# mrvollger/rustybam

Hardware: AMD Instinct MI355X
Metric: CIGAR-ops/s, liftover over 100 kb sliding windows (whole pass, inputs resident in HBM) (higher is better)
Workload: dtype u32

## Files before the change

### rustybam_amd/csrc/capi.hip

```cpp
#include <hip/hip_runtime.h>
#include <sys/mman.h>

#include <algorithm>
#include <cstdarg>
#include <cstdio>
#include <cstdlib>
#include <cstring>
#include <ctime>
#include <numeric>
#include <string>
#include <thread>
#include <vector>
#include <chrono>
#include <map>
#include <mutex>

#include "../../include/rustybam_amd.h"
#include "rb_lift.h"
#include "rb_trim.h"
#include "rb_launch.h"

#ifndef RB_SCAN_ROWS_MEAN_MAX
#define RB_SCAN_ROWS_MEAN_MAX 1536
#endif
#ifndef RB_SHORT_MAX_DEFAULT
#define RB_SHORT_MAX_DEFAULT 2048
#endif

#define RB_MAX_ARENA 256

#define RB_TIMING_RING 256
__global__ __launch_bounds__(256) void rb_k_fill_bytes(uint8_t *dst, uint32_t v4, size_t n) {
    const uintptr_t a = (uintptr_t)dst;
    const size_t head = n < 16 ? n : (size_t)((16 - (a & 15)) & 15);
    const size_t body = (n - head) / 16;
    const size_t tail0 = head + body * 16;
    const size_t i = (size_t)blockIdx.x * blockDim.x + threadIdx.x, stride = (size_t)gridDim.x * blockDim.x;
    for (size_t k = i; k < body; k += stride) *reinterpret_cast<uint4 *>(dst + head + k * 16) = make_uint4(v4, v4, v4, v4);
    if (i < head) dst[i] = (uint8_t)v4;
    if (i < n - tail0) dst[tail0 + i] = (uint8_t)v4;
}
extern "C" hipError_t rb_fill_async(void *dst, int value, size_t bytes, hipStream_t stream) {
    if (!bytes) return hipSuccess;
    const uint32_t b = (uint32_t)value & 255u, v4 = b | (b << 8) | (b << 16) | (b << 24);
// ... 22 lines not shown
    bool pin_busy[2] = {false, false};
    unsigned pin_next = 0;
    uint64_t alloc_fallbacks = 0;
    struct cached_buf { void *p; size_t bytes; bool placed; };
    std::vector<cached_buf> cache;
    size_t cache_bytes = 0;
};
#define RB_PIN_CHUNK ((size_t)32 << 20)
#define RB_PIN_MIN ((size_t)8 << 20)

struct rb_plan {
    rb_ctx *ctx = nullptr;
    uint64_t n_rec = 0, n_win = 0, n_ops = 0;
    uint32_t n_contig = 0;
    uint32_t depth = 0;
    uint32_t *sched = nullptr, *slot_of = nullptr, *canon_pos = nullptr, *w_orig = nullptr, *ident = nullptr;
    uint64_t *w_st = nullptr, *w_en = nullptr, *wo_st = nullptr, *wo_en = nullptr, *cw_off = nullptr;
    uint8_t *cw_mono = nullptr;
    uint32_t *tiles = nullptr;
    uint32_t n_tiles = 0, stream_end = 0;
};

static int fail(rb_ctx *ctx, int code, const char *fmt, ...) {
    if (ctx) {
        char buf[512];
        va_list ap;
        va_start(ap, fmt);
        vsnprintf(buf, sizeof buf, fmt, ap);
        va_end(ap);
        ctx->err = buf;
    }
// ... 496 lines not shown

extern "C" int rb_plan_create(rb_ctx *ctx, uint64_t n_rec, const uint64_t *op_off, const uint32_t *contig, uint64_t n_win,
                              const uint32_t *w_contig, const uint64_t *w_st, const uint64_t *w_en, rb_plan **out) {
    if (!ctx || !out || (n_rec && (!op_off || !contig))) return RB_E_INVALID;
    if (n_rec >= 0xFFFFFFFFull || n_win >= 0xFFFFFFFFull) return fail(ctx, RB_E_INVALID, "too many records/windows for one batch");
    HIPCHK(ctx, hipSetDevice(ctx->device));
    rb_plan *pl = new rb_plan();
    pl->ctx = ctx;
    pl->n_rec = n_rec;
    pl->n_win = n_win;
    uint32_t maxc = 0;
    for (uint64_t i = 0; i < n_rec; i++) maxc = std::max(maxc, contig[i]);
    for (uint64_t i = 0; i < n_win; i++) maxc = std::max(maxc, w_contig[i]);
    const uint32_t n_contig = (n_rec || n_win) ? maxc + 1 : 0;
    pl->n_contig = n_contig;
    std::vector<uint32_t> canon_pos(n_rec);
    {
        std::vector<uint64_t> rank(n_contig, UINT64_MAX);
        uint64_t nr = 0;
        for (uint64_t i = 0; i < n_rec; i++)
            if (rank[contig[i]] == UINT64_MAX) rank[contig[i]] = nr++;
        std::vector<uint64_t> start(nr + 1, 0);
        for (uint64_t i = 0; i < n_rec; i++) start[rank[contig[i]] + 1]++;
        for (uint64_t k = 0; k < nr; k++) start[k + 1] += start[k];
        for (uint64_t i = 0; i < n_rec; i++) canon_pos[i] = (uint32_t)start[rank[contig[i]]]++;
    }
    std::vector<uint32_t> sched(n_rec), ident(n_rec);
    std::iota(ident.begin(), ident.end(), 0u);
    {
        uint64_t max_len = 0;
        std::vector<uint64_t> key(n_rec);
        for (uint64_t i = 0; i < n_rec; i++) key[i] = op_off[i + 1] - op_off[i], max_len = std::max(max_len, key[i]);
        int passes = 0;
        while (passes < 4 && (max_len >> (16 * passes)) != 0) passes++;
        std::vector<uint32_t> a(ident), b(n_rec);
        std::vector<uint64_t> cnt(65537);
        for (int ps = 0; ps < passes; ps++) {
            std::fill(cnt.begin(), cnt.end(), 0);
            const int sh = 16 * ps;
            for (uint64_t i = 0; i < n_rec; i++) cnt[(0xFFFFu - (uint32_t)((key[i] >> sh) & 0xFFFFu)) + 1]++;
// ... 43 lines not shown
        if (const char *m = getenv("RB_SHORT_MAX")) short_max = strtoull(m, nullptr, 10);
        if (on && n_rec) {
            uint64_t n_long = 0;
            rb_cut_tiles(n_rec, op_off, short_max, sched, tiles, &n_long);
            if (!tiles.empty()) pl->stream_end = (uint32_t)n_long;
        }
        pl->n_tiles = (uint32_t)(tiles.size() / 3);
    }
    int rc = RB_OK;
    std::vector<uint32_t> slot_of(n_rec);
    for (uint64_t w = 0; w < n_rec; w++) slot_of[sched[w]] = (uint32_t)w;
    if (!rc) rc = upload_vec(ctx, sched, &pl->sched);
    if (!rc) rc = upload_vec(ctx, slot_of, &pl->slot_of);
    if (!rc) rc = upload_vec(ctx, ident, &pl->ident);
    if (!rc) rc = upload_vec(ctx, canon_pos, &pl->canon_pos);
    if (!rc) rc = upload_vec(ctx, g_st, &pl->w_st);
    if (!rc) rc = upload_vec(ctx, g_en, &pl->w_en);
    if (!rc) rc = upload_vec(ctx, g_orig, &pl->w_orig);
    if (!rc) rc = upload_vec(ctx, o_st, &pl->wo_st);
    if (!rc) rc = upload_vec(ctx, o_en, &pl->wo_en);
    if (!rc) rc = upload_vec(ctx, cw_off, &pl->cw_off);
    if (!rc) rc = upload_vec(ctx, mono, &pl->cw_mono);
    if (!rc && pl->n_tiles) rc = upload_vec(ctx, tiles, &pl->tiles);
    if (!rc && hipStreamSynchronize(ctx->stream) != hipSuccess) rc = fail(ctx, RB_E_HIP, "plan upload: %s", hipGetErrorString(hipGetLastError()));
    if (rc) {
        rb_plan_destroy(pl);
        return rc;
    }
    *out = pl;
    return RB_OK;
}
extern "C" void rb_plan_destroy(rb_plan *pl) {
    if (!pl) return;
    void *ptrs[] = {pl->sched, pl->slot_of, pl->ident, pl->canon_pos, pl->w_st, pl->w_en, pl->w_orig, pl->wo_st, pl->wo_en, pl->cw_off, pl->cw_mono, pl->tiles};
    for (void *q : ptrs)
        if (q) (void)rb_dev_free(pl->ctx, q);
    delete pl;
}

struct ws_layout {
    size_t hit_off, win_lo, block_sums, arena, pend_count, pend_list, jobs, gen_list, x_st, x_en, bp_tmp, bp_off, bp_cur, brk_rows, copy_count, copy_list, decl_count, decl_list, gen_cp, diag_stamps, fb_count, fb_list, starts_bad, total;
};
static bool rb_no_gen_cp() {
    static const bool v = getenv("RB_DEBUG_NO_GEN_CP") != nullptr;
    return v;
}
static ws_layout ws_of(uint64_t n_rec, uint64_t rows_cap, uint64_t n_ops) {
    ws_layout w;
    size_t o = 0;
    auto take = [&](size_t bytes) {
        size_t at = o;
        o += (bytes + 255) & ~(size_t)255;
        return at;
    };
    w.hit_off = take((n_rec + 2) * 8);
    w.win_lo = take((n_rec + 2) * 4);
// ... 6 lines not shown
    w.x_st = take((rows_cap + 1) * 8);
    w.x_en = take((rows_cap + 1) * 8);
    w.bp_tmp = take((rows_cap + 1) * 8);
    w.bp_off = take((n_rec + 1) * 8);
    w.bp_cur = take((size_t)RB_MAX_ARENA * 128);
    w.brk_rows = take((rows_cap + 1) * sizeof(rb_hit_row));
    w.copy_count = take(256);
    w.copy_list = take((rows_cap + 1) * 16);
    w.decl_count = take(256);
    w.decl_list = take((n_rec + 1) * 4);
    w.gen_cp = take(rb_no_gen_cp() ? 256 : (size_t)(n_ops / RB_GCP + n_rec + 2) * sizeof(uint4));
    w.diag_stamps = take((n_rec + 1) * 4);
    w.fb_count = take(256);
    w.fb_list = take((n_rec + 1) * 4);
    w.starts_bad = take(256);
    w.total = o;
    return w;
}
extern "C" size_t rb_plan_workspace_bytes(const rb_plan *plan, uint64_t rows_cap) {
    if (!plan) return 0;
    return ws_of(plan->n_rec, rows_cap, plan->n_ops).total;
}
extern "C" size_t rb_plan_diag_stamps_offset(const rb_plan *plan, uint64_t rows_cap) {
    if (!plan) return 0;
    return ws_of(plan->n_rec, rows_cap, plan->n_ops).diag_stamps;
}

static uint64_t slot_stride_of(uint64_t n_ops, uint64_t n_rec) { return ((n_ops + 31) & ~(uint64_t)31) + 32 * n_rec + 64; }
extern "C" uint64_t rb_plan_out_capacity(const rb_plan *plan, int for_break) {
    if (!plan) return 0;
// ... 76 lines not shown
        HIPCHK(ctx, hipMemcpyAsync(&first_bad, bad, 8, hipMemcpyDeviceToHost, ctx->stream));
        HIPCHK(ctx, hipStreamSynchronize(ctx->stream));
        if (first_bad != ~0ull)
            return fail(ctx, RB_E_INVALID, "RB_LIFT_OP_STARTS: record %llu lies outside the batch's %llu ops (a pass moved it: gather the batch first)",
                        first_bad, (unsigned long long)b->n_ops);
    }
    p.norm_w = const_cast<rb_norm_row *>(norm);
    p.pend_list = (uint32_t *)(ws + w.pend_list);
    p.pend_count = (unsigned long long *)(ws + w.pend_count);
    const bool use_tiles = plan->n_tiles != 0 && ((policy >> 8) & 0xFFF) == 0;
    p.tile_first = use_tiles ? plan->tiles : nullptr;
    p.n_tiles = use_tiles ? plan->n_tiles : 0;
    p.fb_list = (uint32_t *)(ws + w.fb_list);
    p.fb_count = (unsigned long long *)(ws + w.fb_count);
    const uint32_t stream_end = use_tiles ? plan->stream_end : (uint32_t)b->n_rec;
    rb_scan_params sp;
    memset(&sp, 0, sizeof sp);
    if (p.fused) {
        sp.n_rec = b->n_rec;
        sp.ops = b->ops;
        sp.op_off = b->op_off;
        sp.t_st = b->t_st, sp.t_en = b->t_en, sp.q_st = b->q_st, sp.q_en = b->q_en;
        sp.strand = b->strand;
        sp.norm_rows = p.norm_w;
        HIPCHK(ctx, rb_fill_async(p.pend_count, 0, 8, ctx->stream));
        HIPCHK(ctx, rb_launch_peek_norm(&sp, ctx->stream));
    }
    p.counters = counters;
    p.policy = policy & 1;
    p.early_exit = (policy & RB_LIFT_EARLY_EXIT) ? 1 : 0;
    p.debug_skip = (policy >> 8) & 0xFFF;
    uint64_t *block_sums = (uint64_t *)(ws + w.block_sums);
    HIPCHK(ctx, rb_fill_async(counters, 0, sizeof(rb_counters), ctx->stream));
    HIPCHK(ctx, rb_fill_async(p.copy_count, 0, 8, ctx->stream));
    HIPCHK(ctx, rb_fill_async(p.arena_cur, 0, (size_t)RB_MAX_ARENA * RB_ARENA_STRIDE * 8, ctx->stream));
    if (b->n_rec == 0) return RB_OK;
    const bool one_walk = is_break && (policy & RB_BREAK_ONE_WALK) && !p.desc_mode;
    if (one_walk) {
        p.brk_mode = 1, p.brk_max = max_size;
        p.rows_final = rows;
        p.rows = (rb_hit_row *)(ws + w.brk_rows);
        p.brk_off = (uint64_t *)(ws + w.bp_off);
        p.brk_cursor = (unsigned long long *)(ws + w.bp_cur);
        p.brk_n_arena = pick_arenas(b->n_rec);
        p.brk_arena_cap = rows_cap / p.brk_n_arena;
        p.brk_decl_list = (uint32_t *)(ws + w.decl_list);
        p.brk_decl_count = (unsigned long long *)(ws + w.decl_count);
        HIPCHK(ctx, rb_fill_async(p.brk_decl_count, 0, 8, ctx->stream));
        HIPCHK(ctx, rb_fill_async(p.brk_cursor, 0, (size_t)RB_MAX_ARENA * 128, ctx->stream));
        HIPCHK(ctx, rb_fill_async(p.hit_off, 0, (size_t)(b->n_rec + 2) * 8, ctx->stream));
        HIPCHK(ctx, rb_fill_async(p.brk_off, 0xFF, (size_t)(b->n_rec + 1) * 8, ctx->stream));
        HIPCHK(ctx, rb_launch_make_jobs(&p, ctx->stream));
        const size_t slot1 = (size_t)(ctx->timed_calls % RB_TIMING_RING);
        if (ctx->timing) HIPCHK(ctx, hipEventRecord(ctx->ev_a[slot1], ctx->stream));
        p.wave0 = 0;
        p.wave_end = stream_end;
        HIPCHK(ctx, rb_launch_liftover_stream(&p, ctx->stream));
        if (use_tiles) {
            HIPCHK(ctx, rb_fill_async(p.fb_count, 0, 8, ctx->stream));
            HIPCHK(ctx, rb_launch_liftover_tiles(&p, ctx->stream));
            HIPCHK(ctx, rb_launch_liftover_stream_list(&p, ctx->stream));
        }
        if (p.fused) {
            sp.list = p.pend_list;
            sp.n_list = (const uint64_t *)p.pend_count;
            HIPCHK(ctx, rb_launch_scan_records(&sp, ctx->stream));
        }
// ... 34 lines not shown
        bp.max_size = max_size;
        bp.tmp = (uint2 *)(ws + w.bp_tmp);
        bp.tmp_off = (uint64_t *)(ws + w.bp_off);
        bp.tmp_cursor = (unsigned long long *)(ws + w.bp_cur);
        bp.n_arena = pick_arenas(b->n_rec);
        bp.arena_cap = rows_cap / bp.n_arena;
        HIPCHK(ctx, rb_fill_async(bp.tmp_cursor, 0, (size_t)RB_MAX_ARENA * 128, ctx->stream));
        bp.fill = 2, bp.redo_only = 0;
        HIPCHK(ctx, rb_launch_break_pieces(&bp, ctx->stream));
        HIPCHK(ctx, rb_launch_count_and_scan(&p, block_sums, false, ctx->stream));
        HIPCHK(ctx, rb_launch_break_place(&bp, ctx->stream));
        bp.fill = 1, bp.redo_only = 1;
        HIPCHK(ctx, rb_launch_break_pieces(&bp, ctx->stream));
        p.x_st = bp.x_st;
        p.x_en = bp.x_en;
    } else {
        HIPCHK(ctx, rb_launch_count_and_scan(&p, block_sums, true, ctx->stream));
    }
    HIPCHK(ctx, rb_launch_make_jobs(&p, ctx->stream));
    const size_t slot = (size_t)(ctx->timed_calls % RB_TIMING_RING);
    if (ctx->timing) HIPCHK(ctx, hipEventRecord(ctx->ev_a[slot], ctx->stream));
    p.wave0 = 0;
    p.wave_end = stream_end;
    HIPCHK(ctx, rb_launch_liftover_stream(&p, ctx->stream));
    if (use_tiles) {
        HIPCHK(ctx, rb_fill_async(p.fb_count, 0, 8, ctx->stream));
        HIPCHK(ctx, rb_launch_liftover_tiles(&p, ctx->stream));
        HIPCHK(ctx, rb_launch_liftover_stream_list(&p, ctx->stream));
    }
    if (p.fused) {
        sp.list = p.pend_list;
        sp.n_list = (const uint64_t *)p.pend_count;
        HIPCHK(ctx, rb_launch_scan_records(&sp, ctx->stream));
    }
// ... 1036 lines not shown
```

### rustybam_amd/csrc/k_liftover.hip

```cpp
#include "rb_lift.h"
#include "rb_launch.h"
#include <type_traits>
#include <algorithm>

#define RB_PHASE(i)                                                                                                  \
    if (dbg & 32) {                                                                                                  \
        const long long t_now = clock64();                                                                           \
        if (lane == 0 && (wave & 15) == 0) atomicAdd(&p.counters->phase[i], (uint32_t)((t_now - t_prev) >> 4));       \
        t_prev = t_now;                                                                                              \
    }

#ifndef RB_LIST_TU
__global__ __launch_bounds__(256) void rb_k_count_hits(rb_lift_params p) {
    const uint64_t r = (uint64_t)blockIdx.x * blockDim.x + threadIdx.x;
    if (r >= p.n_rec) return;
    uint64_t cnt = 0;
    const rb_norm_row *nr = &p.norm[r];
    const uint32_t c = p.contig[r];
    if (nr->status == RB_ST_OK && c < p.n_contig) {
        const uint64_t ws = p.cw_off[c], we = p.cw_off[c + 1];
        const uint64_t t_st = nr->t_st, t_en = nr->t_en;
        if (p.cw_mono[c]) {
            const uint64_t lo = rb_lower_en_gt(p.w_en, ws, we, t_st);
            const uint64_t hi = rb_lower_st_ge(p.w_st, ws, we, t_en);
            cnt = hi > lo ? hi - lo : 0;
            p.win_lo[r] = (uint32_t)lo;
        } else {
            for (uint64_t i = ws; i < we; i++) cnt += (t_en > p.w_st[i] && t_st < p.w_en[i]) ? 1 : 0;
        }
    }
    p.hit_off[p.canon_pos[r]] = cnt;
}

#define RB_SCAN_PER_BLOCK 2048
__global__ __launch_bounds__(256) void rb_k_scan_partial(const uint64_t *v, uint64_t n, uint64_t *block_sums) {
    __shared__ uint64_t sh[4];
    const uint64_t base = (uint64_t)blockIdx.x * RB_SCAN_PER_BLOCK;
    uint64_t s = 0;
    for (int k = 0; k < RB_SCAN_PER_BLOCK / 256; k++) {
        uint64_t i = base + (uint64_t)k * 256 + threadIdx.x;
        if (i < n) s += v[i];
    }
    s = rb_wave_sum_u64(s);
    if ((threadIdx.x & 63) == 0) sh[threadIdx.x >> 6] = s;
// ... 48 lines not shown
    for (int k = 0; k < RB_SCAN_PER_BLOCK / 256; k++) {
        if (i0 + k < n) v[i0 + k] = run;
        run += x[k];
    }
    if (blockIdx.x == gridDim.x - 1 && threadIdx.x == 255) {
        const uint64_t total = block_sums[gridDim.x];
        v[n] = total;
        if (total_out) *total_out = total;
    }
}

__global__ __launch_bounds__(256) void rb_k_make_jobs(rb_lift_params p) {
    const uint64_t r64 = (uint64_t)blockIdx.x * blockDim.x + threadIdx.x;
    if (r64 >= p.n_rec) return;
    const uint32_t r = (uint32_t)r64;
    const uint64_t w = p.slot_of[r];
    const rb_norm_row *nr = &p.norm[r];
    rb_job j;
    j.r = r;
    j.n = nr->n_ops;
    j.rec0 = p.op_off[r] + nr->first_op;
    j.t_st = nr->t_st, j.t_en = nr->t_en, j.q_st = nr->q_st, j.q_en = nr->q_en;
    const uint64_t k = p.canon_pos[r];
    const bool brk = p.brk_mode != 0;
    const uint64_t h0 = brk ? 0ull : p.hit_off[k], nh = brk ? 1ull : p.hit_off[k + 1] - h0;
    const bool explicit_w = brk || p.x_st != nullptr;
    const uint32_t cg = p.contig[r];
    const bool mono = explicit_w || (cg < p.n_contig && p.cw_mono[cg] != 0);
    uint32_t f = 0;
    const bool provisional = (nr->flags & RB_F_PROVISIONAL) != 0;
    if (nr->status == RB_ST_OK && (nh != 0 || provisional)) {
        if (h0 + nh > p.rows_cap) f |= RB_JOB_ROWS_OVERFLOW;
        else f |= RB_JOB_VALID;
    }
    if ((nr->flags & RB_F_REGULAR) || (provisional && !(nr->flags & RB_F_ENDS_NOT_MATCH))) f |= RB_JOB_REGULAR;
    if (p.strand[r] == (uint8_t)'-') f |= RB_JOB_MINUS;
    if (mono) f |= RB_JOB_MONO;
    j.flags = f;
    j.h0 = (uint32_t)h0;
    j.nh = (uint32_t)nh;
    j.lo = (explicit_w || !mono || !(f & RB_JOB_VALID) || nh == 0) ? 0u : p.win_lo[r];
    p.jobs[w] = j;
}

#endif
#ifndef RB_OPL
#define RB_OPL 8
#endif
static_assert(RB_OPL == 8 || RB_OPL == 4, "ops per lane and step: 8 or 4");
#define RB_GRP (RB_OPL / 4)
#define RB_STEP_SHIFT (RB_OPL == 8 ? 9 : 8)
#define RB_CP_PER_STEP ((64 * RB_OPL) / RB_CP_OPS)
#define RB_CP_LANES (RB_CP_OPS / RB_OPL)
#ifndef RB_PF
#define RB_PF (RB_OPL == 8 ? 2 : 4)
#endif
#ifndef RB_SEG
// ... 1839 lines not shown
```

### rustybam_amd/csrc/k_records.hip

```cpp
#include "rb_device.h"
#include "rb_launch.h"
#include <algorithm>
#include <type_traits>

struct rb_strip {
    uint32_t lead, trail;
    uint64_t dR, dQ;
    uint64_t t_st, t_en, q_st, q_en;
};
__device__ __forceinline__ rb_strip rb_strip_ends(const uint32_t *ops, uint64_t n, uint64_t t_st, uint64_t t_en, uint64_t q_st, uint64_t q_en,
                                                  bool minus) {
    rb_strip o;
    uint64_t lead = 0, rm_st_t = 0, rm_st_q = 0;
    uint32_t prev = RB_NULL_OP;
    o.dR = o.dQ = 0;
    while (lead < n) {
        uint32_t opc, len;
        const uint32_t words = rb_op_fwd(ops, n, lead, &opc, &len);
        if (!rb_in(RB_INDEL_MASK, opc)) break;
        if (opc == RB_OP_D) {
            rm_st_t += len;
            rm_st_q += 1;
            o.dR += len;
        } else {
// ... 21 lines not shown
        }
        trail += words;
    }
    o.lead = (uint32_t)lead;
    o.trail = (uint32_t)trail;
    o.t_st = t_st + rm_st_t, o.t_en = t_en - rm_en_t;
    if (minus) {
        const uint64_t t = rm_st_q;
        rm_st_q = rm_en_q;
        rm_en_q = t;
    }
    o.q_st = q_st + rm_st_q, o.q_en = q_en - rm_en_q;
    return o;
}

__global__ __launch_bounds__(256) void rb_k_peek_norm(rb_scan_params p) {
    const uint64_t r = (uint64_t)blockIdx.x * blockDim.x + threadIdx.x;
    if (r >= p.n_rec) return;
    const uint64_t o0 = p.op_off[r], n = p.op_off[r + 1] - o0;
    rb_norm_row w;
    w.t_st = w.t_en = w.q_st = w.q_en = 0;
    w.first_op = w.n_ops = w.lead_ops = w.trail_ops = w.nmatch = w.aln_len = 0;
    w.flags = RB_F_PROVISIONAL;
    uint32_t st = RB_ST_OK;
    if (n == 0) {
        st = RB_ST_PANIC_EMPTY_CIGAR;
    } else {
        const bool minus = p.strand && p.strand[r] == (uint8_t)'-';
        const rb_strip sp = rb_strip_ends(p.ops + o0, n, p.t_st[r], p.t_en[r], p.q_st[r], p.q_en[r], minus);
        w.lead_ops = sp.lead;
        w.trail_ops = sp.trail;
        if (sp.lead || sp.trail) w.flags |= RB_F_STRIPPED;
        if ((uint64_t)sp.lead + sp.trail > n) {
            st = RB_ST_PANIC_ALL_INDEL;
        } else {
            w.t_st = sp.t_st, w.t_en = sp.t_en, w.q_st = sp.q_st, w.q_en = sp.q_en;
            w.first_op = sp.lead;
            w.n_ops = (uint32_t)(n - sp.lead - sp.trail);
            const uint32_t fo = rb_opc(p.ops[o0 + sp.lead]), lo_ = rb_opc(p.ops[o0 + n - 1 - sp.trail]);
            if (fo > 8u || lo_ > 8u || !rb_in(RB_MATCH_MASK, fo) || !rb_in(RB_MATCH_MASK, lo_)) w.flags |= RB_F_ENDS_NOT_MATCH;
        }
    }
    if (st != RB_ST_OK) w.flags &= ~(uint32_t)RB_F_PROVISIONAL;
    w.status = st;
    p.norm_rows[r] = w;
}

__device__ __forceinline__ void rb_scan_finish(const rb_scan_params &p, const uint64_t r, const uint64_t (&L)[9], const uint32_t ins_events,
                                               const uint32_t del_events, const uint32_t bad, const uint64_t o0, const uint64_t o1, const uint64_t t_st,
                                               const uint64_t t_en, const uint64_t q_st, const uint64_t q_en, const bool minus) {
    const uint64_t n = o1 - o0;
    const uint64_t R = L[RB_OP_M] + L[RB_OP_D] + L[RB_OP_N] + L[RB_OP_EQ] + L[RB_OP_X];
    const uint64_t Q = L[RB_OP_M] + L[RB_OP_I] + L[RB_OP_S] + L[RB_OP_EQ] + L[RB_OP_X];
    const uint64_t M = L[RB_OP_M] + L[RB_OP_EQ] + L[RB_OP_X];
    uint64_t U = 0;
#pragma unroll
    for (int t = 0; t < 9; t++) U += L[t];
    uint32_t flags = 0;
    if (bad == 0 && U <= 0xFFFFFFFFull) flags |= RB_F_REGULAR;
    if (L[RB_OP_M] != 0) flags |= RB_F_HAS_M;
// ... 292 lines not shown
    {
        const unsigned long long h = hist[RB_OP_H][lane], q = hist[RB_OP_P][lane];
        const uint32_t s_lo = rb_row_sum(((uint32_t)h & 0xFFFFFu) + ((uint32_t)q & 0xFFFFFu));
        const uint32_t s_hi = rb_row_sum(((uint32_t)(h >> 20) & 0xFFFFFu) + ((uint32_t)(q >> 20) & 0xFFFFFu));
        L[RB_OP_H] = (uint64_t)s_lo + ((uint64_t)s_hi << 20);
        L[RB_OP_P] = 0;
    }
    const uint32_t ins_events = rb_row_sum((uint32_t)(hist[RB_OP_I][lane] >> RB_LEN_BITS));
    const uint32_t del_events = rb_row_sum((uint32_t)(hist[RB_OP_D][lane] >> RB_LEN_BITS));
    uint32_t bad = (v_reg != 0xFFFFFFFFu ? 1u : 0u) | (v_minlen == 0u ? 2u : 0u) | (v_adj == 0u ? 4u : 0u) | v_big;
    bad = (rb_row_ballot((bad & 1u) != 0u, gbase) ? 1u : 0u) | (rb_row_ballot((bad & 2u) != 0u, gbase) ? 2u : 0u) |
          (rb_row_ballot((bad & 4u) != 0u, gbase) ? 4u : 0u) | (rb_row_ballot((bad & 8u) != 0u, gbase) ? 8u : 0u);
    if (take && gl == 0u) rb_scan_finish(p, r, L, ins_events, del_events, bad, o0, o1, t_st, t_en, q_st, q_en, minus);
}

extern "C" hipError_t rb_launch_peek_norm(const rb_scan_params *p, hipStream_t stream) {
    if (p->n_rec == 0) return hipSuccess;
    hipLaunchKernelGGL(rb_k_peek_norm, dim3((unsigned)((p->n_rec + 255) / 256)), dim3(256), 0, stream, *p);
    return hipGetLastError();
}
extern "C" hipError_t rb_launch_scan_records(const rb_scan_params *p, hipStream_t stream) {
    if (p->n_rec == 0) return hipSuccess;
    const uint64_t blocks = p->list ? std::min<uint64_t>((p->n_rec + 3) / 4, 1024) : (p->n_rec + 3) / 4;
    hipLaunchKernelGGL(rb_k_scan_records, dim3((unsigned)blocks), dim3(256), 0, stream, *p);
    return hipGetLastError();
}
extern "C" hipError_t rb_launch_scan_rows(const rb_scan_params *p, void *long_buf, hipStream_t stream) {
    if (p->n_rec == 0) return hipSuccess;
    unsigned long long *n_long = (unsigned long long *)long_buf;
    uint32_t *long_list = (uint32_t *)((char *)long_buf + 256);
// ... 8 lines not shown
```

### rustybam_amd/csrc/rb_launch.h

```cpp
#pragma once
#include <hip/hip_runtime.h>
#include <stdint.h>

#include "../../include/rustybam_amd.h"

struct rb_lift_params;
struct rb_trim_params;
struct nf_read;
struct nf_tdesc;

struct rb_scan_params {
    uint64_t n_rec;
    const uint32_t *ops;
    const uint64_t *op_off;
    const uint64_t *t_st, *t_en, *q_st, *q_en;
    const uint8_t *strand;
    rb_reduce_row *reduce_rows;
    rb_norm_row *norm_rows;
    const uint32_t *list;
    const uint64_t *n_list;
};
extern "C" hipError_t rb_launch_scan_records(const rb_scan_params *p, hipStream_t stream);
extern "C" hipError_t rb_launch_scan_rows(const rb_scan_params *p, void *long_buf, hipStream_t stream);
extern "C" hipError_t rb_launch_peek_norm(const rb_scan_params *p, hipStream_t stream);

extern "C" hipError_t rb_launch_count_and_scan(const rb_lift_params *p, uint64_t *block_sums, bool do_count, hipStream_t stream);
extern "C" hipError_t rb_launch_exclusive_scan(uint64_t *v, uint64_t n, uint64_t *block_sums, uint64_t *total_out, hipStream_t stream);
extern "C" size_t rb_scan_block_sums_count(uint64_t n_rec);
extern "C" hipError_t rb_launch_make_jobs(const rb_lift_params *p, hipStream_t stream);
extern "C" hipError_t rb_launch_liftover_stream(const rb_lift_params *p, hipStream_t stream);
extern "C" hipError_t rb_launch_liftover_tail(const rb_lift_params *p, hipStream_t stream);
extern "C" hipError_t rb_launch_liftover_stream_list(const rb_lift_params *p, hipStream_t stream);
extern "C" hipError_t rb_launch_liftover_tiles(const rb_lift_params *p, hipStream_t stream);
extern "C" uint32_t rb_tile_max_ops(void);
extern "C" uint32_t rb_tile_max_records(void);
extern "C" hipError_t rb_launch_break_gather(const rb_lift_params *p, hipStream_t stream);
extern "C" hipError_t rb_launch_break_declined(const rb_lift_params *p, hipStream_t stream);
extern "C" hipError_t rb_launch_break_list_declined(const rb_lift_params *p, hipStream_t stream);

// ... 154 lines not shown
```

### rustybam_amd/csrc/rb_lift.h

```cpp
#pragma once
#include "rb_device.h"
#include <cstdlib>


#define RB_HMAX 32
#define RB_LDS_PER_HIT 6
#define RB_ARENA_STRIDE 16
#ifndef RB_MS
#define RB_MS 2
#endif

struct __attribute__((aligned(64))) rb_job {
    uint64_t rec0;
    uint32_t n;
    uint32_t r;
    uint32_t h0;
    uint32_t flags;
    uint32_t nh;
    uint32_t lo;
    uint64_t t_st, t_en, q_st, q_en;
};
enum { RB_JOB_VALID = 1, RB_JOB_REGULAR = 2, RB_JOB_MINUS = 4, RB_JOB_MONO = 8, RB_JOB_ROWS_OVERFLOW = 16 };

struct rb_lift_params {
// ... 78 lines not shown
__device__ __forceinline__ uint64_t rb_lower_en_gt(const uint64_t *w_en, uint64_t lo, uint64_t hi, uint64_t t_st) {
    while (lo < hi) {
        uint64_t mid = lo + ((hi - lo) >> 1);
        if (w_en[mid] > t_st) hi = mid; else lo = mid + 1;
    }
    return lo;
}
__device__ __forceinline__ uint64_t rb_lower_st_ge(const uint64_t *w_st, uint64_t lo, uint64_t hi, uint64_t t_en) {
    while (lo < hi) {
        uint64_t mid = lo + ((hi - lo) >> 1);
        if (w_st[mid] >= t_en) hi = mid; else lo = mid + 1;
    }
    return lo;
}

enum { RB_S_UNRES = 0, RB_S_OK = 1, RB_S_NONE = 2, RB_S_DEFER = 3 };

__device__ __forceinline__ int rb_ffs64(unsigned long long m) { return __ffsll((long long)m) - 1; }

__device__ inline void rb_defer_record(rb_kparams kp, uint32_t r, const rb_norm_row *nr, uint64_t h0, uint64_t nh,
                                bool explicit_w, bool mono, uint64_t ws, uint64_t we, int lane) {
    asm volatile("" : "+v"(lane));
    const rb_kparams q_ = rb_kp_here(kp);
    struct { const uint64_t *w_st, *w_en; const uint32_t *w_orig; rb_hit_row *rows; uint64_t rows_cap; uint32_t *gen_list; rb_counters *counters; } p =
        {q_->w_st, q_->w_en, q_->w_orig, q_->rows, q_->rows_cap, q_->gen_list, q_->counters};
    if (explicit_w || mono) {
        uint64_t lo = 0;
        if (!explicit_w) lo = rb_lower_en_gt(p.w_en, ws, we, nr->t_st);
        for (uint64_t j = lane; j < nh; j += 64) {
            const uint64_t h = h0 + j;
// ... 220 lines not shown
```

Measured before the change: 531.1 billion.

## Fuse lift setup into one kernel with decoupled look-back scan

Replaces the sequence of fill kernels, peek_norm, count_and_scan and make_jobs with a single rb_k_lift_setup kernel. That kernel zeroes counters and arenas, normalises records with a fast path for plain CIGAR ends, counts window hits using interleaved binary searches, computes the hit-offset prefix sum through a single-pass decoupled look-back, and emits jobs. Records are processed in canonical order through a new canon_rec array so the hit offsets come out contiguous. The goal is to cut launch overhead and extra global-memory passes. In exchange it relies on forward progress between blocks through the atomic ticket and look-back spinning, and on a spin limit that raises an overflow flag.

```diff
diff --git a/rustybam_amd/csrc/capi.hip b/rustybam_amd/csrc/capi.hip
--- a/rustybam_amd/csrc/capi.hip
+++ b/rustybam_amd/csrc/capi.hip
@@ -26,8 +26,6 @@
 #ifndef RB_SHORT_MAX_DEFAULT
 #define RB_SHORT_MAX_DEFAULT 2048
 #endif
-
-#define RB_MAX_ARENA 256
 
 #define RB_TIMING_RING 256
 __global__ __launch_bounds__(256) void rb_k_fill_bytes(uint8_t *dst, uint32_t v4, size_t n) {
@@ -80,7 +78,7 @@
     uint64_t n_rec = 0, n_win = 0, n_ops = 0;
     uint32_t n_contig = 0;
     uint32_t depth = 0;
-    uint32_t *sched = nullptr, *slot_of = nullptr, *canon_pos = nullptr, *w_orig = nullptr, *ident = nullptr;
+    uint32_t *sched = nullptr, *slot_of = nullptr, *canon_pos = nullptr, *canon_rec = nullptr, *w_orig = nullptr, *ident = nullptr;
     uint64_t *w_st = nullptr, *w_en = nullptr, *wo_st = nullptr, *wo_en = nullptr, *cw_off = nullptr;
     uint8_t *cw_mono = nullptr;
     uint32_t *tiles = nullptr;
@@ -607,7 +605,7 @@
     for (uint64_t i = 0; i < n_win; i++) maxc = std::max(maxc, w_contig[i]);
     const uint32_t n_contig = (n_rec || n_win) ? maxc + 1 : 0;
     pl->n_contig = n_contig;
-    std::vector<uint32_t> canon_pos(n_rec);
+    std::vector<uint32_t> canon_pos(n_rec), canon_rec(n_rec);
     {
         std::vector<uint64_t> rank(n_contig, UINT64_MAX);
         uint64_t nr = 0;
@@ -617,6 +615,7 @@
         for (uint64_t i = 0; i < n_rec; i++) start[rank[contig[i]] + 1]++;
         for (uint64_t k = 0; k < nr; k++) start[k + 1] += start[k];
         for (uint64_t i = 0; i < n_rec; i++) canon_pos[i] = (uint32_t)start[rank[contig[i]]]++;
+        for (uint64_t i = 0; i < n_rec; i++) canon_rec[canon_pos[i]] = (uint32_t)i;
     }
     std::vector<uint32_t> sched(n_rec), ident(n_rec);
     std::iota(ident.begin(), ident.end(), 0u);
@@ -690,6 +689,7 @@
     if (!rc) rc = upload_vec(ctx, slot_of, &pl->slot_of);
     if (!rc) rc = upload_vec(ctx, ident, &pl->ident);
     if (!rc) rc = upload_vec(ctx, canon_pos, &pl->canon_pos);
+    if (!rc) rc = upload_vec(ctx, canon_rec, &pl->canon_rec);
     if (!rc) rc = upload_vec(ctx, g_st, &pl->w_st);
     if (!rc) rc = upload_vec(ctx, g_en, &pl->w_en);
     if (!rc) rc = upload_vec(ctx, g_orig, &pl->w_orig);
@@ -708,14 +708,14 @@
 }
 extern "C" void rb_plan_destroy(rb_plan *pl) {
     if (!pl) return;
-    void *ptrs[] = {pl->sched, pl->slot_of, pl->ident, pl->canon_pos, pl->w_st, pl->w_en, pl->w_orig, pl->wo_st, pl->wo_en, pl->cw_off, pl->cw_mono, pl->tiles};
+    void *ptrs[] = {pl->sched, pl->slot_of, pl->ident, pl->canon_pos, pl->canon_rec, pl->w_st, pl->w_en, pl->w_orig, pl->wo_st, pl->wo_en, pl->cw_off, pl->cw_mono, pl->tiles};
     for (void *q : ptrs)
         if (q) (void)rb_dev_free(pl->ctx, q);
     delete pl;
 }
 
 struct ws_layout {
-    size_t hit_off, win_lo, block_sums, arena, pend_count, pend_list, jobs, gen_list, x_st, x_en, bp_tmp, bp_off, bp_cur, brk_rows, copy_count, copy_list, decl_count, decl_list, gen_cp, diag_stamps, fb_count, fb_list, starts_bad, total;
+    size_t hit_off, win_lo, block_sums, arena, pend_count, pend_list, jobs, gen_list, x_st, x_en, bp_tmp, bp_off, bp_cur, brk_rows, copy_count, copy_list, decl_count, decl_list, gen_cp, diag_stamps, fb_count, fb_list, starts_bad, setup_lb, total;
 };
 static bool rb_no_gen_cp() {
     static const bool v = getenv("RB_DEBUG_NO_GEN_CP") != nullptr;
@@ -752,6 +752,7 @@
     w.fb_count = take(256);
     w.fb_list = take((n_rec + 1) * 4);
     w.starts_bad = take(256);
+    w.setup_lb = take(rb_setup_state_words(n_rec) * 8);
     w.total = o;
     return w;
 }
@@ -858,6 +859,8 @@
     p.fb_list = (uint32_t *)(ws + w.fb_list);
     p.fb_count = (unsigned long long *)(ws + w.fb_count);
     const uint32_t stream_end = use_tiles ? plan->stream_end : (uint32_t)b->n_rec;
+    const bool one_walk = is_break && (policy & RB_BREAK_ONE_WALK) && !p.desc_mode;
+    const bool setup1 = (!is_break || one_walk) && b->n_rec != 0;
     rb_scan_params sp;
     memset(&sp, 0, sizeof sp);
     if (p.fused) {
@@ -867,19 +870,26 @@
         sp.t_st = b->t_st, sp.t_en = b->t_en, sp.q_st = b->q_st, sp.q_en = b->q_en;
         sp.strand = b->strand;
         sp.norm_rows = p.norm_w;
-        HIPCHK(ctx, rb_fill_async(p.pend_count, 0, 8, ctx->stream));
-        HIPCHK(ctx, rb_launch_peek_norm(&sp, ctx->stream));
+        if (!setup1) {
+            HIPCHK(ctx, rb_fill_async(p.pend_count, 0, 8, ctx->stream));
+            HIPCHK(ctx, rb_launch_peek_norm(&sp, ctx->stream));
+        }
     }
     p.counters = counters;
     p.policy = policy & 1;
     p.early_exit = (policy & RB_LIFT_EARLY_EXIT) ? 1 : 0;
     p.debug_skip = (policy >> 8) & 0xFFF;
     uint64_t *block_sums = (uint64_t *)(ws + w.block_sums);
-    HIPCHK(ctx, rb_fill_async(counters, 0, sizeof(rb_counters), ctx->stream));
-    HIPCHK(ctx, rb_fill_async(p.copy_count, 0, 8, ctx->stream));
-    HIPCHK(ctx, rb_fill_async(p.arena_cur, 0, (size_t)RB_MAX_ARENA * RB_ARENA_STRIDE * 8, ctx->stream));
+    if (!setup1) {
+        HIPCHK(ctx, rb_fill_async(counters, 0, sizeof(rb_counters), ctx->stream));
+        HIPCHK(ctx, rb_fill_async(p.copy_count, 0, 8, ctx->stream));
+        HIPCHK(ctx, rb_fill_async(p.arena_cur, 0, (size_t)RB_MAX_ARENA * RB_ARENA_STRIDE * 8, ctx->stream));
+    }
     if (b->n_rec == 0) return RB_OK;
-    const bool one_walk = is_break && (policy & RB_BREAK_ONE_WALK) && !p.desc_mode;
+    rb_setup_params su;
+    su.canon_rec = is_break ? plan->ident : plan->canon_rec;
+    su.t_st = b->t_st, su.t_en = b->t_en, su.q_st = b->q_st, su.q_en = b->q_en;
+    su.lb = (unsigned long long *)(ws + w.setup_lb);
     if (one_walk) {
         p.brk_mode = 1, p.brk_max = max_size;
         p.rows_final = rows;
@@ -890,11 +900,7 @@
         p.brk_arena_cap = rows_cap / p.brk_n_arena;
         p.brk_decl_list = (uint32_t *)(ws + w.decl_list);
         p.brk_decl_count = (unsigned long long *)(ws + w.decl_count);
-        HIPCHK(ctx, rb_fill_async(p.brk_decl_count, 0, 8, ctx->stream));
-        HIPCHK(ctx, rb_fill_async(p.brk_cursor, 0, (size_t)RB_MAX_ARENA * 128, ctx->stream));
-        HIPCHK(ctx, rb_fill_async(p.hit_off, 0, (size_t)(b->n_rec + 2) * 8, ctx->stream));
-        HIPCHK(ctx, rb_fill_async(p.brk_off, 0xFF, (size_t)(b->n_rec + 1) * 8, ctx->stream));
-        HIPCHK(ctx, rb_launch_make_jobs(&p, ctx->stream));
+        HIPCHK(ctx, rb_launch_lift_setup(&p, &su, ctx->stream));
         const size_t slot1 = (size_t)(ctx->timed_calls % RB_TIMING_RING);
         if (ctx->timing) HIPCHK(ctx, hipEventRecord(ctx->ev_a[slot1], ctx->stream));
         p.wave0 = 0;
@@ -959,10 +965,10 @@
         HIPCHK(ctx, rb_launch_break_pieces(&bp, ctx->stream));
         p.x_st = bp.x_st;
         p.x_en = bp.x_en;
+        HIPCHK(ctx, rb_launch_make_jobs(&p, ctx->stream));
     } else {
-        HIPCHK(ctx, rb_launch_count_and_scan(&p, block_sums, true, ctx->stream));
-    }
-    HIPCHK(ctx, rb_launch_make_jobs(&p, ctx->stream));
+        HIPCHK(ctx, rb_launch_lift_setup(&p, &su, ctx->stream));
+    }
     const size_t slot = (size_t)(ctx->timed_calls % RB_TIMING_RING);
     if (ctx->timing) HIPCHK(ctx, hipEventRecord(ctx->ev_a[slot], ctx->stream));
     p.wave0 = 0;
diff --git a/rustybam_amd/csrc/k_liftover.hip b/rustybam_amd/csrc/k_liftover.hip
--- a/rustybam_amd/csrc/k_liftover.hip
+++ b/rustybam_amd/csrc/k_liftover.hip
@@ -14,20 +14,13 @@
 __global__ __launch_bounds__(256) void rb_k_count_hits(rb_lift_params p) {
     const uint64_t r = (uint64_t)blockIdx.x * blockDim.x + threadIdx.x;
     if (r >= p.n_rec) return;
+    const rb_norm_row *nr = &p.norm[r];
     uint64_t cnt = 0;
-    const rb_norm_row *nr = &p.norm[r];
-    const uint32_t c = p.contig[r];
-    if (nr->status == RB_ST_OK && c < p.n_contig) {
-        const uint64_t ws = p.cw_off[c], we = p.cw_off[c + 1];
-        const uint64_t t_st = nr->t_st, t_en = nr->t_en;
-        if (p.cw_mono[c]) {
-            const uint64_t lo = rb_lower_en_gt(p.w_en, ws, we, t_st);
-            const uint64_t hi = rb_lower_st_ge(p.w_st, ws, we, t_en);
-            cnt = hi > lo ? hi - lo : 0;
-            p.win_lo[r] = (uint32_t)lo;
-        } else {
-            for (uint64_t i = ws; i < we; i++) cnt += (t_en > p.w_st[i] && t_st < p.w_en[i]) ? 1 : 0;
-        }
+    if (nr->status == RB_ST_OK) {
+        uint32_t lo;
+        bool mono;
+        cnt = rb_count_hits(p, p.contig[r], nr->t_st, nr->t_en, &lo, &mono);
+        if (mono) p.win_lo[r] = lo;
     }
     p.hit_off[p.canon_pos[r]] = cnt;
 }
@@ -106,33 +99,10 @@
     const uint64_t r64 = (uint64_t)blockIdx.x * blockDim.x + threadIdx.x;
     if (r64 >= p.n_rec) return;
     const uint32_t r = (uint32_t)r64;
-    const uint64_t w = p.slot_of[r];
-    const rb_norm_row *nr = &p.norm[r];
-    rb_job j;
-    j.r = r;
-    j.n = nr->n_ops;
-    j.rec0 = p.op_off[r] + nr->first_op;
-    j.t_st = nr->t_st, j.t_en = nr->t_en, j.q_st = nr->q_st, j.q_en = nr->q_en;
     const uint64_t k = p.canon_pos[r];
     const bool brk = p.brk_mode != 0;
     const uint64_t h0 = brk ? 0ull : p.hit_off[k], nh = brk ? 1ull : p.hit_off[k + 1] - h0;
-    const bool explicit_w = brk || p.x_st != nullptr;
-    const uint32_t cg = p.contig[r];
-    const bool mono = explicit_w || (cg < p.n_contig && p.cw_mono[cg] != 0);
-    uint32_t f = 0;
-    const bool provisional = (nr->flags & RB_F_PROVISIONAL) != 0;
-    if (nr->status == RB_ST_OK && (nh != 0 || provisional)) {
-        if (h0 + nh > p.rows_cap) f |= RB_JOB_ROWS_OVERFLOW;
-        else f |= RB_JOB_VALID;
-    }
-    if ((nr->flags & RB_F_REGULAR) || (provisional && !(nr->flags & RB_F_ENDS_NOT_MATCH))) f |= RB_JOB_REGULAR;
-    if (p.strand[r] == (uint8_t)'-') f |= RB_JOB_MINUS;
-    if (mono) f |= RB_JOB_MONO;
-    j.flags = f;
-    j.h0 = (uint32_t)h0;
-    j.nh = (uint32_t)nh;
-    j.lo = (explicit_w || !mono || !(f & RB_JOB_VALID) || nh == 0) ? 0u : p.win_lo[r];
-    p.jobs[w] = j;
+    p.jobs[p.slot_of[r]] = rb_job_of(p, r, p.norm[r], h0, nh, [&]() { return p.win_lo[r]; });
 }
 
 #endif
diff --git a/rustybam_amd/csrc/k_records.hip b/rustybam_amd/csrc/k_records.hip
--- a/rustybam_amd/csrc/k_records.hip
+++ b/rustybam_amd/csrc/k_records.hip
@@ -1,4 +1,4 @@
-#include "rb_device.h"
+#include "rb_lift.h"
 #include "rb_launch.h"
 #include <algorithm>
 #include <type_traits>
@@ -59,10 +59,8 @@
     return o;
 }
 
-__global__ __launch_bounds__(256) void rb_k_peek_norm(rb_scan_params p) {
-    const uint64_t r = (uint64_t)blockIdx.x * blockDim.x + threadIdx.x;
-    if (r >= p.n_rec) return;
-    const uint64_t o0 = p.op_off[r], n = p.op_off[r + 1] - o0;
+__device__ __forceinline__ rb_norm_row rb_peek_row(const uint32_t *ops, uint64_t o0, uint64_t n, uint64_t t_st, uint64_t t_en, uint64_t q_st,
+                                                   uint64_t q_en, bool minus) {
     rb_norm_row w;
     w.t_st = w.t_en = w.q_st = w.q_en = 0;
     w.first_op = w.n_ops = w.lead_ops = w.trail_ops = w.nmatch = w.aln_len = 0;
@@ -71,8 +69,7 @@
     if (n == 0) {
         st = RB_ST_PANIC_EMPTY_CIGAR;
     } else {
-        const bool minus = p.strand && p.strand[r] == (uint8_t)'-';
-        const rb_strip sp = rb_strip_ends(p.ops + o0, n, p.t_st[r], p.t_en[r], p.q_st[r], p.q_en[r], minus);
+        const rb_strip sp = rb_strip_ends(ops + o0, n, t_st, t_en, q_st, q_en, minus);
         w.lead_ops = sp.lead;
         w.trail_ops = sp.trail;
         if (sp.lead || sp.trail) w.flags |= RB_F_STRIPPED;
@@ -82,13 +79,20 @@
             w.t_st = sp.t_st, w.t_en = sp.t_en, w.q_st = sp.q_st, w.q_en = sp.q_en;
             w.first_op = sp.lead;
             w.n_ops = (uint32_t)(n - sp.lead - sp.trail);
-            const uint32_t fo = rb_opc(p.ops[o0 + sp.lead]), lo_ = rb_opc(p.ops[o0 + n - 1 - sp.trail]);
+            const uint32_t fo = rb_opc(ops[o0 + sp.lead]), lo_ = rb_opc(ops[o0 + n - 1 - sp.trail]);
             if (fo > 8u || lo_ > 8u || !rb_in(RB_MATCH_MASK, fo) || !rb_in(RB_MATCH_MASK, lo_)) w.flags |= RB_F_ENDS_NOT_MATCH;
         }
     }
     if (st != RB_ST_OK) w.flags &= ~(uint32_t)RB_F_PROVISIONAL;
     w.status = st;
-    p.norm_rows[r] = w;
+    return w;
+}
+__global__ __launch_bounds__(256) void rb_k_peek_norm(rb_scan_params p) {
+    const uint64_t r = (uint64_t)blockIdx.x * blockDim.x + threadIdx.x;
+    if (r >= p.n_rec) return;
+    const uint64_t o0 = p.op_off[r], n = p.op_off[r + 1] - o0;
+    const bool minus = p.strand && p.strand[r] == (uint8_t)'-';
+    p.norm_rows[r] = rb_peek_row(p.ops, o0, n, p.t_st[r], p.t_en[r], p.q_st[r], p.q_en[r], minus);
 }
 
 __device__ __forceinline__ void rb_scan_finish(const rb_scan_params &p, const uint64_t r, const uint64_t (&L)[9], const uint32_t ins_events,
@@ -411,6 +415,209 @@
     if (take && gl == 0u) rb_scan_finish(p, r, L, ins_events, del_events, bad, o0, o1, t_st, t_en, q_st, q_en, minus);
 }
 
+#define RB_LB_AGG 1ull
+#define RB_LB_INCL 2ull
+#define RB_LB_SPIN_MAX (1u << 24)
+
+typedef __attribute__((address_space(1))) unsigned long long rb_gu64;
+static_assert(offsetof(rb_counters, n_hits) == 0 && sizeof(rb_counters) == 64, "rb_k_lift_setup zeroes the counters word by word, n_hits aside");
+
+__device__ __forceinline__ uint64_t rb_wave_scan_incl_u64(uint64_t v, int lane) {
+#pragma unroll
+    for (int off = 1; off < 64; off <<= 1) {
+        const uint64_t y = __shfl_up(v, (unsigned)off, 64);
+        if (lane >= off) v += y;
+    }
+    return v;
+}
+
+#ifndef RB_SU_R
+#define RB_SU_R 4
+#endif
+
+__device__ __forceinline__ bool rb_peek_plain(uint32_t first, uint32_t last, uint64_t n) {
+    return n != 0 && rb_in(RB_MATCH_MASK, first & 15u) && rb_in(RB_MATCH_MASK, last & 15u);
+}
+
+__global__ __launch_bounds__(256) void rb_k_lift_setup(rb_lift_params p, rb_setup_params s) {
+    __shared__ uint32_t s_ticket;
+    __shared__ uint64_t s_wave[4];
+    __shared__ uint64_t s_base;
+    const bool scan = p.brk_mode == 0;
+    const int lane = rb_lane(), wv = (int)(threadIdx.x >> 6);
+    uint32_t t = blockIdx.x;
+    if (scan) {
+        if (threadIdx.x == 0) s_ticket = (uint32_t)__hip_atomic_fetch_add((rb_gu64 *)s.lb, 1ull, __ATOMIC_RELAXED, __HIP_MEMORY_SCOPE_AGENT);
+        __syncthreads();
+        t = s_ticket;
+    }
+    if (t == 0) {
+        uint32_t *c = (uint32_t *)p.counters;
+        if (threadIdx.x < sizeof(rb_counters) / 4 && !(scan && threadIdx.x < 2)) c[threadIdx.x] = 0;
+        if (threadIdx.x == 0) *p.copy_count = 0;
+        if (threadIdx.x == 1 && p.fused) *p.pend_count = 0;
+        for (uint32_t i = threadIdx.x; i < RB_MAX_ARENA_WORDS; i += 256) p.arena_cur[i] = 0;
+        if (!scan) {
+            if (threadIdx.x == 2) *p.brk_decl_count = 0;
+            for (uint32_t i = threadIdx.x; i < RB_MAX_ARENA_WORDS; i += 256) p.brk_cursor[i] = 0;
+        }
+    }
+    const uint64_t n = p.n_rec;
+    const uint64_t k0 = ((uint64_t)t * 256 + threadIdx.x) * RB_SU_R;
+    uint32_t r[RB_SU_R];
+    rb_norm_row nr[RB_SU_R];
+    uint64_t cnt[RB_SU_R];
+    uint32_t lo[RB_SU_R];
+#pragma unroll
+    for (int j = 0; j < RB_SU_R; j++) r[j] = k0 + j < n ? s.canon_rec[k0 + j] : 0u, cnt[j] = 0, lo[j] = 0;
+    if (p.fused) {
+        uint64_t o0[RB_SU_R], no[RB_SU_R];
+        uint32_t fw[RB_SU_R], lw[RB_SU_R];
+#pragma unroll
+        for (int j = 0; j < RB_SU_R; j++) o0[j] = p.op_off[r[j]], no[j] = p.op_off[r[j] + 1] - o0[j];
+#pragma unroll
+        for (int j = 0; j < RB_SU_R; j++) {
+            fw[j] = no[j] ? p.ops[o0[j]] : 0u;
+            lw[j] = no[j] ? p.ops[o0[j] + no[j] - 1] : 0u;
+        }
+#pragma unroll
+        for (int j = 0; j < RB_SU_R; j++) {
+            if (k0 + j >= n) continue;
+            const uint32_t rj = r[j];
+            if (rb_peek_plain(fw[j], lw[j], no[j])) {
+                rb_norm_row &w = nr[j];
+                w.t_st = s.t_st[rj], w.t_en = s.t_en[rj], w.q_st = s.q_st[rj], w.q_en = s.q_en[rj];
+                w.first_op = 0, w.n_ops = (uint32_t)no[j], w.lead_ops = w.trail_ops = w.nmatch = w.aln_len = 0;
+                w.flags = RB_F_PROVISIONAL, w.status = RB_ST_OK;
+            } else {
+                const bool minus = p.strand && p.strand[rj] == (uint8_t)'-';
+                nr[j] = rb_peek_row(p.ops, o0[j], no[j], s.t_st[rj], s.t_en[rj], s.q_st[rj], s.q_en[rj], minus);
+            }
+            p.norm_w[rj] = nr[j];
+        }
+    } else {
+#pragma unroll
+        for (int j = 0; j < RB_SU_R; j++)
+            if (k0 + j < n) nr[j] = p.norm[r[j]];
+    }
+    uint64_t h0[RB_SU_R], own = 0;
+    if (scan) {
+        uint64_t l1[RB_SU_R], h1[RB_SU_R], l2[RB_SU_R], h2[RB_SU_R], wl[RB_SU_R];
+        bool bs = false;
+#pragma unroll
+        for (int j = 0; j < RB_SU_R; j++) {
+            l1[j] = h1[j] = l2[j] = h2[j] = wl[j] = 0;
+            if (k0 + j >= n || nr[j].status != RB_ST_OK) continue;
+            const uint32_t c = p.contig[r[j]];
+            if (c >= p.n_contig) continue;
+            const uint64_t ws = p.cw_off[c], we = p.cw_off[c + 1];
+            if (p.cw_mono[c]) {
+                l1[j] = l2[j] = ws, h1[j] = h2[j] = we, wl[j] = we;
+                bs = true;
+            } else {
+                for (uint64_t i = ws; i < we; i++) cnt[j] += (nr[j].t_en > p.w_st[i] && nr[j].t_st < p.w_en[i]) ? 1 : 0;
+            }
+        }
+        while (bs) {
+            uint64_t a[RB_SU_R], b[RB_SU_R];
+#pragma unroll
+            for (int j = 0; j < RB_SU_R; j++) {
+                const uint64_t m1 = l1[j] + ((h1[j] - l1[j]) >> 1), m2 = l2[j] + ((h2[j] - l2[j]) >> 1);
+                a[j] = l1[j] < h1[j] ? p.w_en[m1] : 0;
+                b[j] = l2[j] < h2[j] ? p.w_st[m2] : 0;
+            }
+            bs = false;
+#pragma unroll
+            for (int j = 0; j < RB_SU_R; j++) {
+                const uint64_t m1 = l1[j] + ((h1[j] - l1[j]) >> 1), m2 = l2[j] + ((h2[j] - l2[j]) >> 1);
+                if (l1[j] < h1[j]) {
+                    if (a[j] > nr[j].t_st) h1[j] = m1; else l1[j] = m1 + 1;
+                }
+                if (l2[j] < h2[j]) {
+                    if (b[j] >= nr[j].t_en) h2[j] = m2; else l2[j] = m2 + 1;
+                }
+                bs |= l1[j] < h1[j] || l2[j] < h2[j];
+            }
+        }
+#pragma unroll
+        for (int j = 0; j < RB_SU_R; j++) {
+            if (wl[j]) {
+                cnt[j] = l2[j] > l1[j] ? l2[j] - l1[j] : 0;
+                lo[j] = (uint32_t)l1[j];
+            }
+            own += cnt[j];
+        }
+        const uint64_t incl = rb_wave_scan_incl_u64(own, lane);
+        if (lane == 63) s_wave[wv] = incl;
+        __syncthreads();
+        uint64_t before = 0;
+        for (int i = 0; i < wv; i++) before += s_wave[i];
+        const uint64_t agg = s_wave[0] + s_wave[1] + s_wave[2] + s_wave[3];
+        if (wv == 0) {
+            rb_gu64 *lb = (rb_gu64 *)s.lb + 1;
+            uint64_t base = 0;
+            if (t == 0) {
+                if (lane == 0) __hip_atomic_store(&lb[0], (RB_LB_INCL << 62) | agg, __ATOMIC_RELAXED, __HIP_MEMORY_SCOPE_AGENT);
+            } else {
+                if (lane == 0) __hip_atomic_store(&lb[t], (RB_LB_AGG << 62) | agg, __ATOMIC_RELAXED, __HIP_MEMORY_SCOPE_AGENT);
+                int64_t top = (int64_t)t - 1;
+                uint32_t spins = 0;
+                for (;;) {
+                    const int64_t j = top - lane;
+                    const uint64_t x = j >= 0 ? __hip_atomic_load(&lb[j], __ATOMIC_RELAXED, __HIP_MEMORY_SCOPE_AGENT) : (RB_LB_INCL << 62);
+                    const uint64_t fl = x >> 62;
+                    const unsigned long long incl_m = rb_ballot(fl == RB_LB_INCL), none_m = rb_ballot(fl == 0);
+                    const int stop = incl_m ? __ffsll((long long)incl_m) - 1 : 63;
+                    const unsigned long long need = stop == 63 ? ~0ull : ((2ull << stop) - 1);
+                    if (none_m & need) {
+                        if (++spins >= RB_LB_SPIN_MAX) {
+                            if (lane == 0) atomicOr(&p.counters->overflow, 1u);
+                            break;
+                        }
+                        __builtin_amdgcn_s_sleep(1);
+                        continue;
+                    }
+                    base += rb_wave_sum_u64(lane <= stop ? (x & ((1ull << 62) - 1)) : 0ull);
+                    if (incl_m) break;
+                    top -= 64;
+                }
+                if (lane == 0) __hip_atomic_store(&lb[t], (RB_LB_INCL << 62) | (base + agg), __ATOMIC_RELAXED, __HIP_MEMORY_SCOPE_AGENT);
+            }
+            if (lane == 0) s_base = base;
+        }
+        __syncthreads();
+        uint64_t run = s_base + before + incl - own;
+#pragma unroll
+        for (int j = 0; j < RB_SU_R; j++) {
+            h0[j] = run;
+            run += cnt[j];
+            if (k0 + j < n) p.hit_off[k0 + j] = h0[j];
+            if (k0 + j + 1 == n) p.hit_off[n] = p.counters->n_hits = run;
+        }
+    } else {
+#pragma unroll
+        for (int j = 0; j < RB_SU_R; j++) {
+            h0[j] = 0, cnt[j] = 1;
+            if (k0 + j < n) p.hit_off[k0 + j] = 0, p.brk_off[k0 + j] = ~0ull;
+            if (k0 + j + 1 == n) p.hit_off[n] = 0, p.hit_off[n + 1] = 0, p.brk_off[n] = ~0ull;
+        }
+    }
+#pragma unroll
+    for (int j = 0; j < RB_SU_R; j++)
+        if (k0 + j < n) p.jobs[p.slot_of[r[j]]] = rb_job_of(p, r[j], nr[j], h0[j], cnt[j], [&]() { return lo[j]; });
+}
+
+extern "C" size_t rb_setup_state_words(uint64_t n_rec) { return (size_t)((n_rec + 256 * RB_SU_R - 1) / (256 * RB_SU_R) + 1); }
+extern "C" hipError_t rb_launch_lift_setup(const rb_lift_params *p, const rb_setup_params *s, hipStream_t stream) {
+    if (p->n_rec == 0) return hipSuccess;
+    const uint64_t blocks = (p->n_rec + 256 * RB_SU_R - 1) / (256 * RB_SU_R);
+    if (!p->brk_mode) {
+        const hipError_t e = rb_fill_async(s->lb, 0, rb_setup_state_words(p->n_rec) * 8, stream);
+        if (e != hipSuccess) return e;
+    }
+    hipLaunchKernelGGL(rb_k_lift_setup, dim3((unsigned)blocks), dim3(256), 0, stream, *p, *s);
+    return hipGetLastError();
+}
 extern "C" hipError_t rb_launch_peek_norm(const rb_scan_params *p, hipStream_t stream) {
     if (p->n_rec == 0) return hipSuccess;
     hipLaunchKernelGGL(rb_k_peek_norm, dim3((unsigned)((p->n_rec + 255) / 256)), dim3(256), 0, stream, *p);
diff --git a/rustybam_amd/csrc/rb_launch.h b/rustybam_amd/csrc/rb_launch.h
--- a/rustybam_amd/csrc/rb_launch.h
+++ b/rustybam_amd/csrc/rb_launch.h
@@ -23,6 +23,13 @@
 extern "C" hipError_t rb_launch_scan_records(const rb_scan_params *p, hipStream_t stream);
 extern "C" hipError_t rb_launch_scan_rows(const rb_scan_params *p, void *long_buf, hipStream_t stream);
 extern "C" hipError_t rb_launch_peek_norm(const rb_scan_params *p, hipStream_t stream);
+struct rb_setup_params {
+    const uint32_t *canon_rec;
+    const uint64_t *t_st, *t_en, *q_st, *q_en;
+    unsigned long long *lb;
+};
+extern "C" hipError_t rb_launch_lift_setup(const rb_lift_params *p, const rb_setup_params *s, hipStream_t stream);
+extern "C" size_t rb_setup_state_words(uint64_t n_rec);
 
 extern "C" hipError_t rb_launch_count_and_scan(const rb_lift_params *p, uint64_t *block_sums, bool do_count, hipStream_t stream);
 extern "C" hipError_t rb_launch_exclusive_scan(uint64_t *v, uint64_t n, uint64_t *block_sums, uint64_t *total_out, hipStream_t stream);
diff --git a/rustybam_amd/csrc/rb_lift.h b/rustybam_amd/csrc/rb_lift.h
--- a/rustybam_amd/csrc/rb_lift.h
+++ b/rustybam_amd/csrc/rb_lift.h
@@ -6,6 +6,8 @@
 #define RB_HMAX 32
 #define RB_LDS_PER_HIT 6
 #define RB_ARENA_STRIDE 16
+#define RB_MAX_ARENA 256
+#define RB_MAX_ARENA_WORDS (RB_MAX_ARENA * RB_ARENA_STRIDE)
 #ifndef RB_MS
 #define RB_MS 2
 #endif
@@ -116,6 +118,49 @@
     return lo;
 }
 
+__device__ __forceinline__ uint64_t rb_count_hits(const rb_lift_params &p, uint32_t c, uint64_t t_st, uint64_t t_en, uint32_t *lo, bool *mono) {
+    *mono = false;
+    if (c >= p.n_contig) return 0;
+    const uint64_t ws = p.cw_off[c], we = p.cw_off[c + 1];
+    if (p.cw_mono[c]) {
+        const uint64_t l = rb_lower_en_gt(p.w_en, ws, we, t_st);
+        const uint64_t h = rb_lower_st_ge(p.w_st, ws, we, t_en);
+        *lo = (uint32_t)l;
+        *mono = true;
+        return h > l ? h - l : 0;
+    }
+    uint64_t cnt = 0;
+    for (uint64_t i = ws; i < we; i++) cnt += (t_en > p.w_st[i] && t_st < p.w_en[i]) ? 1 : 0;
+    return cnt;
+}
+
+template <typename LoF>
+__device__ __forceinline__ rb_job rb_job_of(const rb_lift_params &p, uint32_t r, const rb_norm_row &nr, uint64_t h0, uint64_t nh, LoF &&lo_of) {
+    rb_job j;
+    j.r = r;
+    j.n = nr.n_ops;
+    j.rec0 = p.op_off[r] + nr.first_op;
+    j.t_st = nr.t_st, j.t_en = nr.t_en, j.q_st = nr.q_st, j.q_en = nr.q_en;
+    const bool brk = p.brk_mode != 0;
+    const bool explicit_w = brk || p.x_st != nullptr;
+    const uint32_t cg = p.contig[r];
+    const bool mono = explicit_w || (cg < p.n_contig && p.cw_mono[cg] != 0);
+    uint32_t f = 0;
+    const bool provisional = (nr.flags & RB_F_PROVISIONAL) != 0;
+    if (nr.status == RB_ST_OK && (nh != 0 || provisional)) {
+        if (h0 + nh > p.rows_cap) f |= RB_JOB_ROWS_OVERFLOW;
+        else f |= RB_JOB_VALID;
+    }
+    if ((nr.flags & RB_F_REGULAR) || (provisional && !(nr.flags & RB_F_ENDS_NOT_MATCH))) f |= RB_JOB_REGULAR;
+    if (p.strand[r] == (uint8_t)'-') f |= RB_JOB_MINUS;
+    if (mono) f |= RB_JOB_MONO;
+    j.flags = f;
+    j.h0 = (uint32_t)h0;
+    j.nh = (uint32_t)nh;
+    j.lo = (explicit_w || !mono || !(f & RB_JOB_VALID) || nh == 0) ? 0u : lo_of();
+    return j;
+}
+
 enum { RB_S_UNRES = 0, RB_S_OK = 1, RB_S_NONE = 2, RB_S_DEFER = 3 };
 
 __device__ __forceinline__ int rb_ffs64(unsigned long long m) { return __ffsll((long long)m) - 1; }
```

Result: no change. 531.2 billion, median of 4 (+0.0%).
